# araffin/robotics-rl-srl

Hardware: NVIDIA B200
Metric: env-steps/sec KukaButtonGymEnv-v0 ground_truth @4096 envs/GPU (higher is better)
Workload: dtype f32

## Files before the change

### include/srl_sim.h

```cpp
#ifndef SRL_SIM_H_
#define SRL_SIM_H_

#include <stddef.h>
#include <stdint.h>

#ifdef __cplusplus
extern "C" {
#endif

#define SRL_SIM_ABI_VERSION 1

typedef struct srl_sim srl_sim;

enum srl_env_kind {
    SRL_ENV_KUKA_BUTTON        = 0,
    SRL_ENV_KUKA_RAND_BUTTON   = 1,
    SRL_ENV_KUKA_2BUTTON       = 2,
    SRL_ENV_KUKA_MOVING_BUTTON = 3,
    SRL_ENV_MOBILE             = 4,
    SRL_ENV_MOBILE_2TARGET     = 5,
    SRL_ENV_MOBILE_1D          = 6,
    SRL_ENV_MOBILE_LINE_TARGET = 7
};

typedef struct srl_cfg {
    uint32_t struct_size;
    int32_t  is_discrete;
    int32_t  random_target;
    int32_t  force_down;
    int32_t  shape_reward;
    int32_t  action_joints;
    int32_t  action_repeat;
    int32_t  max_steps;
    int32_t  solver_iterations;
    int32_t  envs_per_warp;
    int32_t  no_auto_reset;
    float    max_distance;
    float    timestep;
    uint32_t prefetch_resets;
    uint64_t global_env_offset;
} srl_cfg;

enum srl_state_field {
    SRL_F_ROBOT_POS     = 0,
    SRL_F_TARGET_POS    = 1,
    SRL_F_STEP_COUNTER  = 2,
    SRL_F_JOINT_POS     = 3,
    SRL_F_JOINT_VEL     = 4,
    SRL_F_EE_CMD        = 5,
    SRL_F_EE_POS        = 6,
    SRL_F_BUTTON_GLIDER = 7,
    SRL_F_COUNTERS      = 8,
    SRL_F_EPISODE_STATS = 9,
    SRL_F_BUTTON_BASE   = 10,
    SRL_F_TWO_BUTTON    = 11,
    SRL_F_NEXT_RECORD   = 12
};

int srl_sim_abi_version(void);

int srl_sim_create(srl_sim** out, int env_kind, int num_envs, int device, const srl_cfg* cfg,
                   const void* model_blob, size_t model_bytes, uint64_t seed);

int srl_sim_reset(srl_sim* sim, const uint8_t* mask, const double* reset_draws, float* obs_out,
                  void* stream);

int srl_sim_step(srl_sim* sim, const void* actions, const float* noise, float* obs_out,
                 float* rew_out, uint8_t* done_out, float* ep_ret_out, int32_t* ep_len_out,
                 void* stream);

int srl_sim_rollout(srl_sim* sim, int T, const void* actions, const float* noise, float* obs_out,
                    float* rew_out, uint8_t* done_out, float* ep_ret_out, int32_t* ep_len_out,
                    void* stream);

int srl_sim_rollout_host(srl_sim* sim, int T, const void* actions, const float* noise,
                         float* obs_out, float* rew_out, uint8_t* done_out);

int srl_sim_prefetch_resets(srl_sim* sim, void* stream);

typedef struct srl_camera {
    float target[3];
    float distance, yaw, pitch, roll;
    float fov;
} srl_camera;
int srl_sim_render(srl_sim* sim, const srl_camera* camera, int width, int height, uint8_t* rgb_out, void* stream);

int srl_sim_get_state(srl_sim* sim, int field, void* dst, size_t bytes);
int srl_sim_set_state(srl_sim* sim, int field, const void* src, size_t bytes);

// ... 16 lines not shown
```

### robotics-rl-srl_b200/csrc/kuka_kernels.cu

```cuda
#include <stdio.h>
#include <stdlib.h>
#include <string.h>
#include <vector>
#include "common.cuh"
#include "kuka_device.cuh"
#include "render_core.h"

struct KukaDev {
    float4* q[3];
    float4* qd[3];
    float4* misc0;
    float4* misc1;
    float4* tgt;
    float4* grip;
    float4* eepos;
    int4*   cnt;
    int4*   cnt2;
    float4* btn2;
    KukaParams P;
    int epw;
    int coop;
};

struct KukaNext {
    float4* q[3]; float4* qd[3];
    float4 *misc0, *misc1, *tgt, *grip, *eepos;
    int4 *cnt, *cnt2;
    float4* btn2;
    uint8_t* valid;
    int32_t* episode;
    uint8_t* progress;
    int helper;
};

namespace {

constexpr float DELTA_V = 0.03f, DELTA_V_CONTINUOUS = 0.0035f, DELTA_THETA = 0.1f;
constexpr double NOISE_STD = 0.01, NOISE_STD_CONTINUOUS = 0.0001, NOISE_STD_JOINTS = 0.002;
constexpr int N_CONTACTS_BEFORE_TERMINATION = 5, N_STEPS_OUTSIDE_SAFETY_SPHERE = 5000, N_RANDOM_ACTIONS_AT_INIT = 5;

template <bool CG, class T>
KK_DEV T ld_state(const T* p) { return CG ? __ldcg(p) : *p; }

template <bool TWOB, bool CG = false, class Arr = KukaDev>
KK_DEV void env_load(const Arr& d, int i, KukaEnv& e) {
#pragma unroll
    for (int k = 0; k < 3; ++k) {
        const float4 a = ld_state<CG>(d.q[k] + i), b = ld_state<CG>(d.qd[k] + i);
        e.q[4 * k] = a.x; e.q[4 * k + 1] = a.y; e.q[4 * k + 2] = a.z; e.q[4 * k + 3] = a.w;
        e.qd[4 * k] = b.x; e.qd[4 * k + 1] = b.y; e.qd[4 * k + 2] = b.z; e.qd[4 * k + 3] = b.w;
    }
    const float4 m0 = ld_state<CG>(d.misc0 + i), m1 = ld_state<CG>(d.misc1 + i), tg = ld_state<CG>(d.tgt + i), gr = ld_state<CG>(d.grip + i),
                 ep = ld_state<CG>(d.eepos + i);
    const int4 c = ld_state<CG>(d.cnt + i), c2 = ld_state<CG>(d.cnt2 + i);
    e.ee[0] = m0.x; e.ee[1] = m0.y; e.ee[2] = m0.z; e.qb = m0.w;
    e.qdb = m1.x; e.bbx = m1.y; e.bby = m1.z; e.ep_ret = m1.w;
    e.tgt[0] = tg.x; e.tgt[1] = tg.y; e.tgt[2] = tg.z; e.bbz = tg.w;
    e.grip[0] = gr.x; e.grip[1] = gr.y; e.grip[2] = gr.z; e.bspeed = gr.w;
    e.eepos[0] = ep.x; e.eepos[1] = ep.y; e.eepos[2] = ep.z;
    e.counter = c.x; e.n_contacts = c.y; e.n_outside = c.z;
    e.terminated = c.w & 1; e.cbutton = (c.w >> 1) & 1; e.ctable = (c.w >> 2) & 1;
    e.episode = (uint32_t)c2.x; e.total_steps = (uint32_t)c2.y; e.ep_len = c2.z;
    e.by64 = __hiloint2double(c2.w, __float_as_int(ep.w));
    e.qb2 = 0.f; e.qdb2 = 0.f; e.bb2x = 0.f; e.bb2y = 0.f; e.n_contacts2 = 0; e.goal_id = 0; e.cany0 = 0; e.cany1 = 0;
// ... 69 lines not shown
        if (P.random_target) {
            if (d17) { e.bb2x = (float)d17[0]; e.bb2y = (float)d17[1]; }
            else {
                const uint4 r = philox4x32_10(P.seed, genv, e.episode, PHILOX_PURPOSE_RESET0);
                e.bb2x = (float)((double)P.btn_base[0] + (double)P.rand_x * (-1.0 + 2.0 * philox_u01(r.x, r.y)));
                e.bb2y = (float)(-(double)P.btn_base[1] + 0.175 * (-1.0 + philox_u01(r.z, r.w)));
            }
        }
        return;
    }
    if (P.random_target) {
        if (d17) { e.bbx = (float)d17[0]; e.bby = (float)d17[1]; e.by64 = d17[1]; }
        else {
            const uint4 r = philox4x32_10(P.seed, genv, e.episode, PHILOX_PURPOSE_RESET0);
            e.bbx = (float)((double)P.btn_base[0] + (double)P.rand_x * (-1.0 + 2.0 * philox_u01(r.x, r.y)));
            e.by64 = (double)P.btn_base[1] + (double)P.rand_y * (-1.0 + 2.0 * philox_u01(r.z, r.w));
            e.bby = (float)e.by64;
        }
    }
}

template <bool TWOB>
KK_DEV void reset_end(const KukaParams& P, KukaEnv& e) {
    e.tgt[0] = e.bbx; e.tgt[1] = e.bby;
    e.tgt[2] = e.bbz + P.glider_z + e.qb + P.target_h;
    if (TWOB) e.tgt[2] = P.two_tgt_z;
    if (TWOB) { e.n_contacts2 = 0; e.goal_id = 0; }
    e.counter = 0; e.n_contacts = 0; e.n_outside = 0; e.terminated = 0;
    e.ep_ret = 0.f; e.ep_len = 0;
    e.episode += 1;
}

enum { KUKA_OP_ROLLOUT = 0, KUKA_OP_RESET = 1, KUKA_OP_SETTLE = 2, KUKA_OP_PREFETCH = 3 };

#ifdef KK_TIMING
__device__ unsigned long long kk_timing[1 << 16];
#define KK_TIMING_RECORD() do { if (lead) kk_timing[(warp * (COOP ? 8 : 32) + slot) & 0xFFFF] = ((unsigned long long)(clock64() - kk_t0) << 32) | dbgf | (helper ? 1u << 18 : 0u); } while (0)
#else
#define KK_TIMING_RECORD() do { } while (0)
#endif
template <bool JOINTS, bool TWOB, bool PREFETCH = false, bool COOP = false>
__global__ void __launch_bounds__(128, 1) kuka_kernel(const __grid_constant__ KukaDev d, int n, int op, int T,
                                                       const void* __restrict__ actions, const float* __restrict__ noise,
                                                       const uint8_t* __restrict__ mask, const double* __restrict__ draws,
                                                       float* __restrict__ obs, float* __restrict__ rew,
                                                       uint8_t* __restrict__ done, float* __restrict__ ep_ret,
                                                       int32_t* __restrict__ ep_len, float* __restrict__ snap, const KukaNext nx) {
    const int lane = threadIdx.x & 31, warp = (blockIdx.x * blockDim.x + threadIdx.x) >> 5;
#ifdef KK_TIMING
    const long long kk_t0 = clock64(); unsigned dbgf = 0u;
#endif
    const int slot = COOP ? lane >> 2 : lane;
    const int u = COOP ? lane & 3 : 0;
    const bool lead = !COOP || u == 0;
    const unsigned gmask = COOP ? 0xFu << (lane & ~3) : 0u;
    extern __shared__ float4 kc_smem[];
    float* const kc_tab = reinterpret_cast<float*>(kc_smem);
    KcScratch sc;
    sc.b = reinterpret_cast<float*>(kc_smem) + ((KC_CONST_WORDS + 31) / 32) * 32 + (8 * (threadIdx.x >> 5) + (lane >> 2)) * KC_ES;
    if constexpr (COOP) {
        kc_fill_const(d.P, kc_tab, threadIdx.x, blockDim.x);
        __syncthreads();
    }
    int i = -1;
    if (slot < d.epw) { i = warp * d.epw + slot; if (i >= n) i = -1; }
    bool helper = false;
    if constexpr (PREFETCH) {
        if (nx.helper && op == KUKA_OP_ROLLOUT && slot == d.epw && slot < (COOP ? 8 : 32)) {
            int pick = -1;
            if (lead) {
                int best = -1;
                for (int k2 = 0; k2 < d.epw; ++k2) {
                    const int j = warp * d.epw + k2;
                    if (j < n && !reinterpret_cast<volatile const uint8_t*>(nx.valid)[j]) {
                        const int pr = nx.progress[j];
                        if (pr > best) { best = pr; pick = j; }
                    }
                }
            }
            if (COOP) pick = __shfl_sync(gmask, pick, lane & ~3);
            if (pick >= 0) { i = pick; helper = true; op = KUKA_OP_PREFETCH; }
        }
    }
    if (i < 0) return;
    if (op == KUKA_OP_RESET && mask && !mask[i]) return;
    if constexpr (PREFETCH) { if (op == KUKA_OP_PREFETCH && !helper && nx.valid[i]) return; }
    const KukaParams& P = d.P;
    const uint64_t genv = P.env_offset + (uint64_t)i;
    const size_t N = (size_t)n;
    KukaEnv e; KukaKin k; KukaContacts ct;
    env_load<TWOB>(d, i, e);
    int nc_reg = 0;
    if constexpr (PREFETCH) {
        __syncwarp();
    }

    int reset_left = 0;
    bool in_reset = false;
    bool pending = false;
    int rep = 0, t = 0;
    int saved_cb = 0, saved_ct = 0, saved_a0 = 0, saved_a1 = 0;
    float dx = 0.f, dy = 0.f, dz = 0.f;
    float qj[JOINTS ? 7 : 1];
#pragma unroll
    for (int j = 0; j < (JOINTS ? 7 : 1); ++j) qj[j] = 0.f;
    const double* d17 = nullptr;
    if (op == KUKA_OP_RESET) {
        d17 = draws ? draws + (size_t)i * 18 : nullptr;
        reset_begin<TWOB>(P, e, d17, genv);
        in_reset = true; reset_left = N_RANDOM_ACTIONS_AT_INIT;
    } else if (op == KUKA_OP_SETTLE) {
#pragma unroll
        for (int j = 0; j < KK_NB; ++j) { e.q[j] = P.snap_q[j]; e.qd[j] = 0.f; }
        e.ee[0] = P.ee_init[0]; e.ee[1] = P.ee_init[1]; e.ee[2] = P.ee_init[2];
        e.qb = 0.f; e.qdb = 0.f; e.bbx = P.btn_base[0]; e.bby = P.btn_base[1]; e.bbz = P.btn_base[2]; e.bspeed = 0.f; e.by64 = 0.0;
        if (TWOB) { e.qb2 = 0.f; e.qdb2 = 0.f; e.bb2x = P.btn_base[0]; e.bb2y = -P.btn_base[1]; }
        in_reset = true; reset_left = 500;
    }
    bool consumed = false;
    bool partial = false;
    int budget = T;
    if constexpr (PREFETCH) {
        if (op == KUKA_OP_PREFETCH) {
            const int prog = helper ? (int)nx.progress[i] : 0;
            if (prog > 0 && nx.episode[i] == (int)e.episode) {
                env_load<TWOB, true>(nx, i, e);
                in_reset = true; reset_left = N_RANDOM_ACTIONS_AT_INIT - prog;
            } else {
                if (helper && lead) nx.episode[i] = (int)e.episode;
                reset_begin<TWOB>(P, e, nullptr, genv);
                in_reset = true; reset_left = N_RANDOM_ACTIONS_AT_INIT;
            }
        }
    }
    for (;;) {
        if constexpr (COOP) {
            KcKinIn kin;
#pragma unroll
            for (int j = 0; j < KK_NB; ++j) kin.q[j] = e.q[j];
            kin.qb = e.qb; kin.qb2 = e.qb2; kin.bbx = e.bbx; kin.bby = e.bby; kin.bbz = e.bbz; kin.bb2x = e.bb2x; kin.bb2y = e.bb2y;
            __syncwarp(gmask);
            const bool near = kc_kinematics<TWOB>(sc, kc_tab, P, kin, u, gmask);
            e.grip[0] = sc[8 * KC_BS + KB_C]; e.grip[1] = sc[8 * KC_BS + KB_C + 1]; e.grip[2] = sc[8 * KC_BS + KB_C + 2];
            e.eepos[0] = sc[6 * KC_BS + KB_P]; e.eepos[1] = sc[6 * KC_BS + KB_P + 1]; e.eepos[2] = sc[6 * KC_BS + KB_P + 2];
            const int fl = near ? (int)sc[KC_OFF_LINK + 6] : 0;
            e.cbutton = fl & 1; e.ctable = (fl >> 1) & 1;
            if (TWOB) { e.cany0 = (fl >> 2) & 1; e.cany1 = (fl >> 3) & 1; }
            nc_reg = near ? (int)sc[KC_OFF_LINK + 7] : 0;
        } else kuka_fk<true, TWOB>(P, e, k, ct);
        const int new_cb = e.cbutton, new_ct = e.ctable, new_a0 = TWOB ? e.cany0 : 0, new_a1 = TWOB ? e.cany1 : 0;
        if (pending) {
            pending = false;
            const size_t off = (size_t)t * N + (size_t)i;
            const float ddx = e.tgt[0] - e.grip[0], ddy = e.tgt[1] - e.grip[1], ddz = e.tgt[2] - e.grip[2];
            const float distance = sqrtf(ddx * ddx + ddy * ddy + ddz * ddz);
            float reward;
            if (TWOB) {
                const int contact = e.goal_id ? saved_a1 : saved_a0;
                reward = 0.f;
                if (e.goal_id) { e.n_contacts2 += contact; reward = contact ? 1.f : 0.f; }
                else {
                    e.n_contacts += contact;
                    if (e.n_contacts >= N_CONTACTS_BEFORE_TERMINATION) { e.goal_id = 1; e.tgt[0] = e.bb2x; e.tgt[1] = e.bb2y; }
                }
                if (distance > P.max_distance || saved_ct) { reward = -1.f; e.n_outside += 1; } else e.n_outside = 0;
                if (saved_ct || e.n_contacts2 >= N_CONTACTS_BEFORE_TERMINATION || e.n_outside >= N_STEPS_OUTSIDE_SAFETY_SPHERE - 1) e.terminated = 1;
                if (P.shape_reward) {
// ... 13 lines not shown
                if (P.is_discrete) reward = -distance;
                else if (e.terminated && reward > 0.f) reward = 50.f;
                else if (e.terminated && reward < 0.f) reward = -250.f;
                else reward = -distance;
            }
            }
            const bool is_done = e.terminated || e.counter > P.max_steps;
#ifdef KK_TIMING
            if (is_done) dbgf |= 1u << 16;
#endif
            e.ep_ret += reward; e.ep_len += 1;
            if (rew && lead) rew[off] = reward;
            if (done && lead) done[off] = is_done ? 1 : 0;
            if (is_done && lead) {
                if (ep_ret) ep_ret[off] = e.ep_ret;
                if (ep_len) ep_len[off] = e.ep_len;
            }
            if (is_done && P.auto_reset) {
                if constexpr (PREFETCH) {
                    if (op == KUKA_OP_ROLLOUT) {
                        int rec = 0;
                        if (lead && reinterpret_cast<volatile const uint8_t*>(nx.valid)[i]) {
                            __threadfence();
                            rec = reinterpret_cast<volatile const int32_t*>(nx.episode)[i] == (int)e.episode ? 2 : 1;
                        }
                        if (COOP) rec = __shfl_sync(gmask, rec, lane & ~3);
#ifdef KK_TIMING
                        if (rec == 2) dbgf |= 1u << 17;
#endif
                        if (rec == 2) {
                            const uint32_t total_steps = e.total_steps;
                            env_load<TWOB, true>(nx, i, e);
                            e.total_steps = total_steps;
                            __threadfence();
                            if (COOP) __syncwarp(gmask);
                        }
                        if (rec && lead) reinterpret_cast<volatile uint8_t*>(nx.valid)[i] = 0;
                        if (rec == 2) {
                            saved_cb = e.cbutton; saved_ct = e.ctable;
                            if (TWOB) { saved_a0 = e.cany0; saved_a1 = e.cany1; }
                            consumed = true; in_reset = true; reset_left = 0;
                            continue;
                        }
                    }
                }
                d17 = nullptr;
                reset_begin<TWOB>(P, e, nullptr, genv);
                in_reset = true; reset_left = N_RANDOM_ACTIONS_AT_INIT;
                continue;
            }
            if (obs && lead) { float* o = obs + 3 * off; o[0] = e.grip[0] - e.tgt[0]; o[1] = e.grip[1] - e.tgt[1]; o[2] = e.grip[2] - e.tgt[2]; }
            ++t;
        }
        if (in_reset && reset_left == 0) {
            in_reset = false;
            if (op == KUKA_OP_SETTLE) {
                if (lead) {
                    for (int j = 0; j < KK_NB; ++j) { snap[j] = e.q[j]; snap[KK_NB + j] = e.qd[j]; }
                    snap[24] = e.ee[0]; snap[25] = e.ee[1]; snap[26] = e.ee[2]; snap[27] = e.qb; snap[28] = e.qdb;
                }
                return;
            }
            if (!(PREFETCH && consumed)) reset_end<TWOB>(P, e);
            consumed = false;
            if (obs && lead && op != KUKA_OP_PREFETCH) {
                float* o = obs + 3 * (op == KUKA_OP_RESET ? (size_t)i : (size_t)t * N + (size_t)i);
                o[0] = e.grip[0] - e.tgt[0]; o[1] = e.grip[1] - e.tgt[1]; o[2] = e.grip[2] - e.tgt[2];
            }
            if (op == KUKA_OP_ROLLOUT) ++t;
        }
        if (!in_reset && (op != KUKA_OP_ROLLOUT || t >= T)) break;
        bool armed;
        if (in_reset) {
            if (op == KUKA_OP_SETTLE) { dx = dy = dz = 0.f; }
            else reset_action(P, d17, genv, e.episode, N_RANDOM_ACTIONS_AT_INIT - reset_left, dx, dy, dz);
            if (JOINTS) {
#pragma unroll
                for (int j = 0; j < 7; ++j) qj[JOINTS ? j : 0] = P.qinit[j] + dx;
            }
            --reset_left;
            armed = false;
        } else {
            if (rep == 0) {
                const size_t off = (size_t)t * N + (size_t)i;
                float nz;
                if (noise) nz = __ldg(noise + off);
                else {
                    const uint4 r = philox4x32_10(P.seed, genv, e.total_steps, PHILOX_PURPOSE_NOISE);
                    const double u1 = philox_u01(r.x, r.y), u2 = philox_u01(r.z, r.w);
                    nz = (float)((JOINTS ? NOISE_STD_JOINTS : P.is_discrete ? NOISE_STD : NOISE_STD_CONTINUOUS) * sqrt(-2.0 * log(1.0 - u1)) * cos(6.283185307179586 * u2));
                }
                dx = dy = dz = 0.f;
                uint4 ra = make_uint4(0, 0, 0, 0);
                if (!actions) ra = philox4x32_10(P.seed, genv, e.total_steps, PHILOX_PURPOSE_ACTION);
                if (JOINTS) {
                    float a7[7];
                    if (actions) {
// ... 23 lines not shown
                    if (actions) {
                        const float* ap = reinterpret_cast<const float*>(actions) + 3 * off;
                        a0 = __ldg(ap); a1 = __ldg(ap + 1); a2 = __ldg(ap + 2);
                    } else {
                        a0 = (float)((double)ra.x * (2.0 / 4294967296.0) - 1.0);
                        a1 = (float)((double)ra.y * (2.0 / 4294967296.0) - 1.0);
                        a2 = (float)((double)ra.z * (2.0 / 4294967296.0) - 1.0);
                    }
                    const float dv = DELTA_V_CONTINUOUS + nz;
                    dx = a0 * dv; dy = a1 * dv;
                    dz = P.force_down ? -fabsf(a2 * dv) : a2 * dv;
                }
                e.total_steps += 1;
                if (P.moving_button) {
                    if (e.by64 > 0.3 || e.by64 < -0.3) e.bspeed = -e.bspeed;
                    e.by64 = __dadd_rn(e.by64, e.bspeed > 0.f ? 0.001 : -0.001);
                    e.tgt[1] = (float)e.by64;
                    e.bbx = e.tgt[0]; e.bby = e.tgt[1]; e.bbz = e.tgt[2] - P.target_h;
                }
            }
            armed = true;
        }
        if (!JOINTS) apply_ee_delta(P, e, dx, dy, dz);
        saved_cb = new_cb; saved_ct = new_ct; saved_a0 = new_a0; saved_a1 = new_a1;
#ifdef KK_TIMING
        kuka_physics_step<JOINTS, TWOB, COOP>(P, e, k, ct, armed, qj, sc, u, gmask, nc_reg, &dbgf);
#else
        kuka_physics_step<JOINTS, TWOB, COOP>(P, e, k, ct, armed, qj, sc, u, gmask, nc_reg);
#endif
        if constexpr (PREFETCH) { if (helper && --budget <= 0 && reset_left > 0) { partial = true; break; } }
        if (!in_reset) {
            if (e.terminated || e.counter > P.max_steps) { pending = true; rep = 0; }
            else { e.counter += 1; if (++rep == P.action_repeat) { pending = true; rep = 0; } }
        }
    }
    e.cbutton = saved_cb; e.ctable = saved_ct;
    if (TWOB) { e.cany0 = saved_a0; e.cany1 = saved_a1; }
    KK_TIMING_RECORD();
    if constexpr (PREFETCH) {
        if (op == KUKA_OP_PREFETCH) {
            if (!lead) return;
            env_store<TWOB>(nx, i, e);
            if (partial) { nx.progress[i] = (uint8_t)(N_RANDOM_ACTIONS_AT_INIT - reset_left); return; }
            nx.episode[i] = (int)e.episode - 1;
            nx.progress[i] = 0;
            __threadfence();
            reinterpret_cast<volatile uint8_t*>(nx.valid)[i] = 1;
            return;
        }
    }
    if (lead) env_store<TWOB>(d, i, e);
}

template <bool TWOB>
__global__ void kuka_prims_kernel(const __grid_constant__ KukaDev d, int n, float* __restrict__ prims, int* __restrict__ counts) {
    const int i = blockIdx.x * blockDim.x + threadIdx.x;
    if (i >= n) return;
    const KukaParams& P = d.P;
    KukaEnv e; KukaKin k; KukaContacts ct;
    env_load<TWOB>(d, i, e);
    float Rb[KK_NB][9]; f3 pb[KK_NB];
    {
        float R[9] = {1.f, 0.f, 0.f, 0.f, 1.f, 0.f, 0.f, 0.f, 1.f}, R7[9]; f3 p = mk3(P.base[0], P.base[1], P.base[2]), p7 = p;
        for (int t = 0; t < 9; ++t) R7[t] = R[t];
        for (int b = 0; b < KK_NB; ++b) {
            if (b == 10) { for (int t = 0; t < 9; ++t) R[t] = R7[t]; p = p7; }
            const float ox = P.org[b][0], oy = P.org[b][1], oz = P.org[b][2];
            p = mk3(p.x + R[0] * ox + R[1] * oy + R[2] * oz, p.y + R[3] * ox + R[4] * oy + R[5] * oz, p.z + R[6] * ox + R[7] * oy + R[8] * oz);
            float sn, cs; sincosf(e.q[b], &sn, &cs);
            const float t = 1.f - cs, ax = P.axis[b][0], ay = P.axis[b][1], az = P.axis[b][2];
            const float Q[9] = {cs + t * ax * ax, t * ax * ay - sn * az, t * ax * az + sn * ay, t * ax * ay + sn * az, cs + t * ay * ay, t * ay * az - sn * ax,
                                t * ax * az - sn * ay, t * ay * az + sn * ax, cs + t * az * az};
            float B[9], Rn[9];
            for (int r = 0; r < 3; ++r) for (int c = 0; c < 3; ++c) B[3 * r + c] = P.rot[b][3 * r] * Q[c] + P.rot[b][3 * r + 1] * Q[3 + c] + P.rot[b][3 * r + 2] * Q[6 + c];
            for (int r = 0; r < 3; ++r) for (int c = 0; c < 3; ++c) Rn[3 * r + c] = R[3 * r] * B[c] + R[3 * r + 1] * B[3 + c] + R[3 * r + 2] * B[6 + c];
            for (int t2 = 0; t2 < 9; ++t2) { R[t2] = Rn[t2]; Rb[b][t2] = Rn[t2]; }
            pb[b] = p;
            if (b == 7) { for (int t2 = 0; t2 < 9; ++t2) R7[t2] = R[t2]; p7 = p; }
        }
    }
// ... 155 lines not shown

int kuka_alloc(srl_sim* s, const void* blob, size_t bytes) {
    KukaDev* d = new KukaDev();
    memset(d, 0, sizeof(*d));
    s->kuka = d;
    if (!fill_params(blob, bytes, s, d->P)) return 1;
    const size_t N = (size_t)s->n;
    float4** f4[] = {&d->q[0], &d->q[1], &d->q[2], &d->qd[0], &d->qd[1], &d->qd[2], &d->misc0, &d->misc1, &d->tgt, &d->grip, &d->eepos};
    for (float4** p : f4) { SRL_CUDA_OK(cudaMalloc(p, N * sizeof(float4))); SRL_CUDA_OK(cudaMemset(*p, 0, N * sizeof(float4))); }
    SRL_CUDA_OK(cudaMalloc(&d->cnt, N * sizeof(int4))); SRL_CUDA_OK(cudaMemset(d->cnt, 0, N * sizeof(int4)));
    SRL_CUDA_OK(cudaMalloc(&d->cnt2, N * sizeof(int4))); SRL_CUDA_OK(cudaMemset(d->cnt2, 0, N * sizeof(int4)));
    SRL_CUDA_OK(cudaMalloc(&d->btn2, N * sizeof(float4))); SRL_CUDA_OK(cudaMemset(d->btn2, 0, N * sizeof(float4)));
    int sms = 148;
    cudaDeviceGetAttribute(&sms, cudaDevAttrMultiProcessorCount, s->device);
    int epw = s->cfg.envs_per_warp;
    if (epw <= 0) { epw = (int)((N + (size_t)sms * 4 - 1) / ((size_t)sms * 4)); }
    if (epw < 1) epw = 1;
    if (epw > 32) epw = 32;
    d->epw = epw;
    d->coop = epw <= 8 ? 1 : 0;
    if (const char* co = getenv("SRL_KUKA_COOP")) d->coop = (atoi(co) != 0 && epw <= 8) ? 1 : 0;
    float* snap = nullptr;
    SRL_CUDA_OK(cudaMalloc(&snap, 32 * sizeof(float)));
    { const int save_epw = d->epw; d->epw = 1;
      KUKA_LAUNCH(d, 1, 32, 0, 1, KUKA_OP_SETTLE, 0, nullptr, nullptr, nullptr, nullptr, nullptr, nullptr, nullptr, nullptr, nullptr, snap);
      d->epw = save_epw; }
    SRL_CUDA_OK(cudaGetLastError());
    float h[32];
    SRL_CUDA_OK(cudaMemcpy(h, snap, sizeof(h), cudaMemcpyDeviceToHost));
    cudaFree(snap);
    for (int i = 0; i < KK_NB; ++i) { d->P.snap_q[i] = h[i]; d->P.snap_qd[i] = h[KK_NB + i]; }
    d->P.snap_ee[0] = h[24]; d->P.snap_ee[1] = h[25]; d->P.snap_ee[2] = h[26]; d->P.snap_qb = h[27]; d->P.snap_qdb = h[28];
    s->launches += 1;
    if (s->cfg.prefetch_resets && s->auto_reset && !d->P.two_buttons && !d->P.action_joints) {
        KukaNextHost* nh = new KukaNextHost();
        memset(nh, 0, sizeof(*nh));
        s->kuka_next = nh;
        KukaNext& nx = nh->nx;
        float4** g4[] = {&nx.q[0], &nx.q[1], &nx.q[2], &nx.qd[0], &nx.qd[1], &nx.qd[2], &nx.misc0, &nx.misc1, &nx.tgt, &nx.grip, &nx.eepos, &nx.btn2};
        for (float4** p : g4) { SRL_CUDA_OK(cudaMalloc(p, N * sizeof(float4))); SRL_CUDA_OK(cudaMemset(*p, 0, N * sizeof(float4))); }
        SRL_CUDA_OK(cudaMalloc(&nx.cnt, N * sizeof(int4))); SRL_CUDA_OK(cudaMemset(nx.cnt, 0, N * sizeof(int4)));
        SRL_CUDA_OK(cudaMalloc(&nx.cnt2, N * sizeof(int4))); SRL_CUDA_OK(cudaMemset(nx.cnt2, 0, N * sizeof(int4)));
        SRL_CUDA_OK(cudaMalloc(&nx.valid, N)); SRL_CUDA_OK(cudaMemset(nx.valid, 0, N));
        SRL_CUDA_OK(cudaMalloc(&nx.episode, N * sizeof(int32_t))); SRL_CUDA_OK(cudaMemset(nx.episode, 0xff, N * sizeof(int32_t)));
        SRL_CUDA_OK(cudaMalloc(&nx.progress, N)); SRL_CUDA_OK(cudaMemset(nx.progress, 0, N));
        SRL_CUDA_OK(cudaEventCreateWithFlags(&s->pf_ev, cudaEventDisableTiming));
        SRL_CUDA_OK(cudaEventCreateWithFlags(&s->roll_ev, cudaEventDisableTiming));
        nh->enabled = true;
    }
    return 0;
}

void kuka_free(srl_sim* s) {
    KukaDev* d = s->kuka;
    if (!d) return;
    for (int k = 0; k < 3; ++k) { cudaFree(d->q[k]); cudaFree(d->qd[k]); }
    cudaFree(d->misc0); cudaFree(d->misc1); cudaFree(d->tgt); cudaFree(d->grip); cudaFree(d->eepos); cudaFree(d->cnt); cudaFree(d->cnt2); cudaFree(d->btn2);
    delete d;
    s->kuka = nullptr;
    if (KukaNextHost* nh = static_cast<KukaNextHost*>(s->kuka_next)) {
        KukaNext& nx = nh->nx;
        for (int k = 0; k < 3; ++k) { cudaFree(nx.q[k]); cudaFree(nx.qd[k]); }
        cudaFree(nx.misc0); cudaFree(nx.misc1); cudaFree(nx.tgt); cudaFree(nx.grip); cudaFree(nx.eepos); cudaFree(nx.cnt); cudaFree(nx.cnt2);
        cudaFree(nx.btn2); cudaFree(nx.valid); cudaFree(nx.episode); cudaFree(nx.progress);
        delete nh;
        s->kuka_next = nullptr;
        if (s->pf_ev) cudaEventDestroy(s->pf_ev);
        if (s->roll_ev) cudaEventDestroy(s->roll_ev);
    }
}

int kuka_launch_reset(srl_sim* s, const uint8_t* mask, const double* draws, float* obs, cudaStream_t st) {
    KukaDev* d = s->kuka;
    int grid, block; grid_for(s, d, grid, block);
    KUKA_LAUNCH(d, grid, block, st, s->n, KUKA_OP_RESET, 0, nullptr, nullptr, mask, draws, obs, nullptr, nullptr, nullptr, nullptr, nullptr);
    SRL_CUDA_OK(cudaGetLastError());
    return 0;
}

int kuka_launch_rollout(srl_sim* s, int T, const void* actions, const float* noise, float* obs, float* rew, uint8_t* done,
                        float* ep_ret, int32_t* ep_len, cudaStream_t st) {
    KukaDev* d = s->kuka;
    int grid, block; grid_for(s, d, grid, block);
    const KukaNextHost* nh = static_cast<const KukaNextHost*>(s->kuka_next);
    if (nh && nh->enabled) {
        cudaStreamCaptureStatus cap = cudaStreamCaptureStatusNone;
        cudaStreamIsCapturing(st, &cap);
        const bool capturing = cap != cudaStreamCaptureStatusNone;
        if (s->pf_pending && !capturing) { SRL_CUDA_OK(cudaStreamWaitEvent(st, s->pf_ev, 0)); s->pf_pending = false; }
        KukaNext nx = nh->nx;
        nx.helper = 1;
        if (d->coop) SRL_CUDA_OK((kuka_launch_inst<false, false, true, true>(d, grid, block, st, s->n, KUKA_OP_ROLLOUT, T, actions, noise, nullptr, nullptr, obs, rew, done, ep_ret, ep_len, nullptr, nx)));
        else SRL_CUDA_OK((kuka_launch_inst<false, false, true, false>(d, grid, block, st, s->n, KUKA_OP_ROLLOUT, T, actions, noise, nullptr, nullptr, obs, rew, done, ep_ret, ep_len, nullptr, nx)));
        if (!capturing) { SRL_CUDA_OK(cudaEventRecord(s->roll_ev, st)); s->roll_ev_valid = true; }
    }
    else
        KUKA_LAUNCH(d, grid, block, st, s->n, KUKA_OP_ROLLOUT, T, actions, noise, nullptr, nullptr, obs, rew, done, ep_ret, ep_len, nullptr);
// ... 85 lines not shown
        SRL_CUDA_OK(pull(a, d->btn2));
        SRL_CUDA_OK(cudaMemcpy(ia.data(), d->cnt, N * sizeof(int4), cudaMemcpyDeviceToHost));
        SRL_CUDA_OK(cudaMemcpy(ib.data(), d->cnt2, N * sizeof(int4), cudaMemcpyDeviceToHost));
        for (size_t i = 0; i < N; ++i) {
            D[8 * i] = d->P.two_buttons ? ia[i].y : 0; D[8 * i + 1] = d->P.two_buttons ? ib[i].w : 0; D[8 * i + 2] = (ia[i].w >> 5) & 1;
            D[8 * i + 3] = a[i].z; D[8 * i + 4] = a[i].w; D[8 * i + 5] = d->P.btn_base[2]; D[8 * i + 6] = a[i].x; D[8 * i + 7] = a[i].y;
        }
        return 0;
    }
    case SRL_F_EPISODE_STATS: {
        if (!need(2, 8)) return 1;
        SRL_CUDA_OK(pull(b, d->misc1));
        SRL_CUDA_OK(cudaMemcpy(ia.data(), d->cnt2, N * sizeof(int4), cudaMemcpyDeviceToHost));
        for (size_t i = 0; i < N; ++i) { D[2 * i] = b[i].w; D[2 * i + 1] = (double)ia[i].z; }
        return 0;
    }
#ifdef KK_TIMING
    case 99: {
        if (cudaMemcpyFromSymbol(dst, kk_timing, bytes < sizeof(kk_timing) ? bytes : sizeof(kk_timing)) != cudaSuccess) return 1;
        return 0;
    }
#endif
    case SRL_F_NEXT_RECORD: {
        if (!need(3, 4)) return 1;
        const KukaNextHost* nh = static_cast<const KukaNextHost*>(s->kuka_next);
        for (size_t i = 0; i < N; ++i) { I[3 * i] = 0; I[3 * i + 1] = 0; I[3 * i + 2] = -1; }
        if (nh && nh->enabled) {
            std::vector<uint8_t> va(N), pr(N); std::vector<int32_t> ep(N);
            SRL_CUDA_OK(cudaMemcpy(va.data(), nh->nx.valid, N, cudaMemcpyDeviceToHost));
            SRL_CUDA_OK(cudaMemcpy(pr.data(), nh->nx.progress, N, cudaMemcpyDeviceToHost));
            SRL_CUDA_OK(cudaMemcpy(ep.data(), nh->nx.episode, N * sizeof(int32_t), cudaMemcpyDeviceToHost));
            for (size_t i = 0; i < N; ++i) { I[3 * i] = va[i]; I[3 * i + 1] = pr[i]; I[3 * i + 2] = ep[i]; }
        }
        return 0;
    }
    default:
        srl_set_error("get_state: unknown field %d", field);
        return 1;
    }
}

int kuka_set_state(srl_sim* s, int field, const void* src, size_t bytes) {
    KukaDev* d = s->kuka;
    const size_t N = (size_t)s->n;
    SRL_CUDA_OK(cudaDeviceSynchronize());
    auto need = [&](size_t width, size_t elem) { if (bytes != N * width * elem) { srl_set_error("set_state: size mismatch"); return false; } return true; };
    const double* D = (const double*)src; const int32_t* I = (const int32_t*)src;
    std::vector<float4> a(N), b(N), c(N);
    auto pull = [&](std::vector<float4>& v, const float4* p) { return cudaMemcpy(v.data(), p, N * sizeof(float4), cudaMemcpyDeviceToHost); };
    auto push = [&](const std::vector<float4>& v, float4* p) { return cudaMemcpy(p, v.data(), N * sizeof(float4), cudaMemcpyHostToDevice); };
    switch (field) {
    case SRL_F_JOINT_POS: case SRL_F_JOINT_VEL: {
        if (!need(KK_NB, 8)) return 1;
        float4* const* dst = field == SRL_F_JOINT_POS ? d->q : d->qd;
        for (size_t i = 0; i < N; ++i) {
            a[i] = make_float4((float)D[12 * i], (float)D[12 * i + 1], (float)D[12 * i + 2], (float)D[12 * i + 3]);
            b[i] = make_float4((float)D[12 * i + 4], (float)D[12 * i + 5], (float)D[12 * i + 6], (float)D[12 * i + 7]);
            c[i] = make_float4((float)D[12 * i + 8], (float)D[12 * i + 9], (float)D[12 * i + 10], (float)D[12 * i + 11]);
        }
        SRL_CUDA_OK(push(a, dst[0])); SRL_CUDA_OK(push(b, dst[1])); SRL_CUDA_OK(push(c, dst[2]));
        return 0;
    }
    case SRL_F_EE_CMD:
        if (!need(3, 8)) return 1;
        SRL_CUDA_OK(pull(a, d->misc0));
        for (size_t i = 0; i < N; ++i) { a[i].x = (float)D[3 * i]; a[i].y = (float)D[3 * i + 1]; a[i].z = (float)D[3 * i + 2]; }
// ... 37 lines not shown
```

### robotics-rl-srl_b200/rl_baselines/ppo2.py

```python
import json
import os
import time

import numpy as np
import torch
import torch.nn as nn

from srl_sim.vec_env import BatchedSRLVecEnv

PPO2_DEFAULTS = dict(n_steps=128, ent_coef=0.01, learning_rate=2.5e-4, vf_coef=0.5, max_grad_norm=0.5, gamma=0.99, lam=0.95,
                     nminibatches=4, noptepochs=4, cliprange=0.2)


class MlpPolicy(nn.Module):

    def __init__(self, obs_dim, n_actions=None, action_dim=None):
        super().__init__()
        self.discrete = n_actions is not None
        out = n_actions if self.discrete else action_dim

        def tower(last, gain):
            layers = [nn.Linear(obs_dim, 64), nn.Tanh(), nn.Linear(64, 64), nn.Tanh(), nn.Linear(64, last)]
            for m in layers:
                if isinstance(m, nn.Linear):
# ... 57 lines not shown
    def stats(mean, var, count):
        return torch.cat([count.reshape(1), count * mean, count * (var + mean * mean)])
    d = norm.mean.numel()
    s = stats(norm.mean, norm.var, norm.count)
    all_reduce_sum(s)
    s = s - (world - 1) * stats(*prior)
    count, mean = s[0], s[1:1 + d] / s[0]
    norm.count.copy_(count)
    norm.mean.copy_(mean)
    norm.var.copy_(torch.clamp(s[1 + d:] / count - mean * mean, min=0.0))


def allreduce_mean_gradients(params, dist, world):
    grads = [p.grad for p in params]
    flat = torch.cat([g.reshape(-1) for g in grads])
    dist.all_reduce(flat)
    flat.div_(world)
    off = 0
    for g in grads:
        n = g.numel()
        g.copy_(flat[off:off + n].view_as(g))
        off += n


def train(env_id, num_envs, num_timesteps, seed=0, env_kwargs=None, log_dir=None, device=0, hyperparams=None, verbose=1, cuda_graph=True,
          phase_times=None, fused_act=None, prefetch_resets=None, episode_window=40, fused_update=None):
    hp = dict(PPO2_DEFAULTS); hp.update(hyperparams or {})
    torch.manual_seed(seed)
    env_kwargs = dict(env_kwargs or {})
    dist, rank, world = _dist_world()
    if prefetch_resets is None:
        from srl_sim.backend import default_backend
        prefetch_resets = default_backend(device).on_gpu
    if prefetch_resets:
        env_kwargs["prefetch_resets"] = True
    if env_kwargs.get("srl_model", "ground_truth") != "ground_truth":
        raise ValueError("ppo2.train supports srl_model='ground_truth' only (got %r)" % env_kwargs["srl_model"])
    import types
    from rl_baselines.utils import createTensorEnvs, save_obs_rms
    env = createTensorEnvs(types.SimpleNamespace(env=env_id, num_cpu=num_envs, seed=seed, device=device), env_kwargs=env_kwargs,
                           global_env_offset=rank * num_envs)
    on_gpu = env.backend.on_gpu
    dev = env.backend.torch_device if on_gpu else torch.device("cpu")
    e_obs, e_rew, e_done, e_ep_ret, e_ep_len = [x if on_gpu else torch.from_numpy(x) for x in (env._obs, env._rew, env._done, env._ep_ret, env._ep_len)]
    D = env.observation_space.shape[0]
    if env.is_discrete:
        policy = MlpPolicy(D, n_actions=env.action_space.n).to(dev)
    else:
        policy = MlpPolicy(D, action_dim=env.action_space.shape[0]).to(dev)
    params = list(policy.parameters())
    if dist is not None:
        for p in params:
            dist.broadcast(p.data, 0)
        torch.manual_seed(seed + rank)
    N, T = num_envs, hp["n_steps"]
    graph_update = bool(cuda_graph and on_gpu and dist is None and (T * N) % hp["nminibatches"] == 0)
    if graph_update:
        lr_t = torch.tensor(float(hp["learning_rate"]), device=dev, dtype=torch.float32)
        opt = torch.optim.Adam(params, lr=lr_t, eps=1e-5, capturable=True)
    else:
        opt = torch.optim.Adam(params, lr=hp["learning_rate"], eps=1e-5)
    norm = RunningNorm(D, dev)
    n_updates = max(1, int(num_timesteps) // (N * T * world))
    if log_dir and rank == 0:
        os.makedirs(log_dir, exist_ok=True)
        with open(os.path.join(log_dir, "args.json"), "w") as f:
            json.dump(dict(env=env_id, algo="ppo2", num_cpu=N, num_timesteps=num_timesteps, seed=seed, srl_model="ground_truth", **hp), f)
        with open(os.path.join(log_dir, "env_globals.json"), "w") as f:
# ... 257 lines not shown
```

### robotics-rl-srl_b200/srl_sim/_abi.py

```python
import ctypes
import os
from ctypes import (POINTER, Structure, byref, c_char_p, c_double, c_float, c_int, c_int32,
                    c_size_t, c_uint8, c_uint32, c_uint64, c_void_p)

import numpy as np

ABI_VERSION = 1

ENV_KINDS = {
    "KukaButtonGymEnv-v0": 0,
    "KukaRandButtonGymEnv-v0": 1,
    "Kuka2ButtonGymEnv-v0": 2,
    "KukaMovingButtonGymEnv-v0": 3,
    "MobileRobotGymEnv-v0": 4,
    "MobileRobot2TargetGymEnv-v0": 5,
    "MobileRobot1DGymEnv-v0": 6,
    "MobileRobotLineTargetGymEnv-v0": 7,
}

F_ROBOT_POS, F_TARGET_POS, F_STEP_COUNTER, F_JOINT_POS, F_JOINT_VEL, F_EE_CMD, F_EE_POS, \
    F_BUTTON_GLIDER, F_COUNTERS, F_EPISODE_STATS, F_BUTTON_BASE, F_TWO_BUTTON, F_NEXT_RECORD = range(13)

_FIELD_SPEC = {
    F_ROBOT_POS: (np.float64, 3), F_TARGET_POS: (np.float64, 3), F_STEP_COUNTER: (np.int32, 1),
    F_JOINT_POS: (np.float64, 12), F_JOINT_VEL: (np.float64, 12), F_EE_CMD: (np.float64, 3),
    F_EE_POS: (np.float64, 3), F_BUTTON_GLIDER: (np.float64, 2), F_COUNTERS: (np.int32, 4),
    F_EPISODE_STATS: (np.float64, 2), F_BUTTON_BASE: (np.float64, 3), F_TWO_BUTTON: (np.float64, 8), F_NEXT_RECORD: (np.int32, 3),
}

MOBILE_RESET_DRAWS = 6
KUKA_RESET_DRAWS = 18


class SrlCfg(Structure):
    _fields_ = [
        ("struct_size", c_uint32),
        ("is_discrete", c_int32),
        ("random_target", c_int32),
        ("force_down", c_int32),
        ("shape_reward", c_int32),
        ("action_joints", c_int32),
        ("action_repeat", c_int32),
        ("max_steps", c_int32),
        ("solver_iterations", c_int32),
        ("envs_per_warp", c_int32),
        ("no_auto_reset", c_int32),
        ("max_distance", c_float),
        ("timestep", c_float),
        ("prefetch_resets", c_uint32),
        ("global_env_offset", c_uint64),
    ]


class SimError(RuntimeError):
    pass


_EXPORTS = [
    ("srl_sim_abi_version", c_int, []),
    ("srl_sim_create", c_int, [POINTER(c_void_p), c_int, c_int, c_int, POINTER(SrlCfg), c_void_p, c_size_t, c_uint64]),
    ("srl_sim_reset", c_int, [c_void_p, c_void_p, c_void_p, c_void_p, c_void_p]),
# ... 55 lines not shown
        return msg.decode("utf-8", "replace") if msg else ""

    def check(self, rc, what):
        if rc != 0:
            msg = self.last_error()
            if rc == 2:
                raise ValueError(msg)
            raise SimError("%s failed (rc=%d): %s" % (what, rc, msg))


class Sim(object):

    def __init__(self, library, env_kind, num_envs, device, seed=0, model_blob=None, **cfg):
        self.library = library
        self._lib = library.lib
        self.handle = c_void_p()
        if isinstance(env_kind, str):
            env_kind = ENV_KINDS[env_kind]
        self.env_kind = env_kind
        c = SrlCfg()
        c.struct_size = ctypes.sizeof(SrlCfg)
        c.is_discrete = int(cfg.pop("is_discrete", True))
        c.random_target = int(cfg.pop("random_target", False))
        c.force_down = int(cfg.pop("force_down", True))
        c.shape_reward = int(cfg.pop("shape_reward", False))
        c.action_joints = int(cfg.pop("action_joints", False))
        c.action_repeat = int(cfg.pop("action_repeat", 1))
        c.max_steps = int(cfg.pop("max_steps", 0))
        c.solver_iterations = int(cfg.pop("solver_iterations", 0))
        c.envs_per_warp = int(cfg.pop("envs_per_warp", 0))
        c.no_auto_reset = int(cfg.pop("no_auto_reset", False))
        c.max_distance = float(cfg.pop("max_distance", 0.8))
        c.timestep = float(cfg.pop("timestep", 0.0))
        c.prefetch_resets = int(bool(cfg.pop("prefetch_resets", False)))
        c.global_env_offset = int(cfg.pop("global_env_offset", 0))
        if cfg:
            raise TypeError("unknown cfg keys: %s" % sorted(cfg))
        self.cfg = c
        blob_ptr, blob_len = None, 0
        if model_blob is not None:
            self._blob = np.ascontiguousarray(model_blob)
            blob_ptr, blob_len = self._blob.ctypes.data, self._blob.nbytes
        rc = self._lib.srl_sim_create(byref(self.handle), env_kind, int(num_envs), int(device), byref(c),
                                      blob_ptr, blob_len, int(seed) & 0xFFFFFFFFFFFFFFFF)
        library.check(rc, "srl_sim_create")
        self.num_envs = self._lib.srl_sim_num_envs(self.handle)
        self.obs_dim = self._lib.srl_sim_obs_dim(self.handle)
        self.action_dim = self._lib.srl_sim_action_dim(self.handle)
        self.is_discrete = bool(c.is_discrete)
        self.device = device

    def close(self):
        if self.handle:
            self._lib.srl_sim_destroy(self.handle)
            self.handle = c_void_p()

    def __del__(self):
        try:
            self.close()
        except Exception:
            pass

    def reset(self, mask=None, reset_draws=None, obs_out=None, stream=None):
        rc = self._lib.srl_sim_reset(self.handle, _ptr(mask), _ptr(reset_draws), _ptr(obs_out), stream)
        self.library.check(rc, "srl_sim_reset")

    def step(self, actions, noise=None, obs_out=None, rew_out=None, done_out=None, ep_ret_out=None,
# ... 59 lines not shown
```

Before: 98.93 million.

## Enable reset prefetch by default, chain helper records, prefetch step inputs to L1

```diff
diff --git a/include/srl_sim.h b/include/srl_sim.h
--- a/include/srl_sim.h
+++ b/include/srl_sim.h
@@ -41,6 +41,8 @@
     uint64_t global_env_offset;
 } srl_cfg;
 
+enum srl_prefetch_mode { SRL_PREFETCH_DEFAULT = 0, SRL_PREFETCH_ON = 1, SRL_PREFETCH_OFF = 2 };
+
 enum srl_state_field {
     SRL_F_ROBOT_POS     = 0,
     SRL_F_TARGET_POS    = 1,
@@ -54,7 +56,8 @@
     SRL_F_EPISODE_STATS = 9,
     SRL_F_BUTTON_BASE   = 10,
     SRL_F_TWO_BUTTON    = 11,
-    SRL_F_NEXT_RECORD   = 12
+    SRL_F_NEXT_RECORD   = 12,
+    SRL_F_RECORD_HITS   = 13
 };
 
 int srl_sim_abi_version(void);
diff --git a/robotics-rl-srl_b200/csrc/kuka_kernels.cu b/robotics-rl-srl_b200/csrc/kuka_kernels.cu
--- a/robotics-rl-srl_b200/csrc/kuka_kernels.cu
+++ b/robotics-rl-srl_b200/csrc/kuka_kernels.cu
@@ -30,6 +30,7 @@
     uint8_t* valid;
     int32_t* episode;
     uint8_t* progress;
+    int32_t* hits;
     int helper;
 };
 
@@ -165,6 +166,30 @@
 }
 
 enum { KUKA_OP_ROLLOUT = 0, KUKA_OP_RESET = 1, KUKA_OP_SETTLE = 2, KUKA_OP_PREFETCH = 3 };
+
+KK_DEV int record_pick(const KukaNext& nx, int warp, int epw, int n) {
+    int pick = -1, best = -1;
+    for (int k2 = 0; k2 < epw; ++k2) {
+        const int j = warp * epw + k2;
+        if (j < n && !reinterpret_cast<volatile const uint8_t*>(nx.valid)[j]) {
+            const int pr = nx.progress[j];
+            if (pr > best) { best = pr; pick = j; }
+        }
+    }
+    if (pick >= 0) __threadfence();
+    return pick;
+}
+
+template <bool TWOB>
+KK_DEV void record_publish(const KukaNext& nx, int i, const KukaEnv& e) {
+    env_store<TWOB>(nx, i, e);
+    nx.episode[i] = (int)e.episode - 1;
+    nx.progress[i] = 0;
+    __threadfence();
+    reinterpret_cast<volatile uint8_t*>(nx.valid)[i] = 1;
+}
+
+KK_DEV void prefetch_l1(const void* p) { asm volatile("prefetch.global.L1 [%0];" ::"l"(p)); }
 
 #ifdef KK_TIMING
 __device__ unsigned long long kk_timing[1 << 16];
@@ -200,17 +225,7 @@
     bool helper = false;
     if constexpr (PREFETCH) {
         if (nx.helper && op == KUKA_OP_ROLLOUT && slot == d.epw && slot < (COOP ? 8 : 32)) {
-            int pick = -1;
-            if (lead) {
-                int best = -1;
-                for (int k2 = 0; k2 < d.epw; ++k2) {
-                    const int j = warp * d.epw + k2;
-                    if (j < n && !reinterpret_cast<volatile const uint8_t*>(nx.valid)[j]) {
-                        const int pr = nx.progress[j];
-                        if (pr > best) { best = pr; pick = j; }
-                    }
-                }
-            }
+            int pick = lead ? record_pick(nx, warp, d.epw, n) : -1;
             if (COOP) pick = __shfl_sync(gmask, pick, lane & ~3);
             if (pick >= 0) { i = pick; helper = true; op = KUKA_OP_PREFETCH; }
         }
@@ -219,7 +234,7 @@
     if (op == KUKA_OP_RESET && mask && !mask[i]) return;
     if constexpr (PREFETCH) { if (op == KUKA_OP_PREFETCH && !helper && nx.valid[i]) return; }
     const KukaParams& P = d.P;
-    const uint64_t genv = P.env_offset + (uint64_t)i;
+    uint64_t genv = P.env_offset + (uint64_t)i;
     const size_t N = (size_t)n;
     KukaEnv e; KukaKin k; KukaContacts ct;
     env_load<TWOB>(d, i, e);
@@ -250,22 +265,37 @@
         if (TWOB) { e.qb2 = 0.f; e.qdb2 = 0.f; e.bb2x = P.btn_base[0]; e.bb2y = -P.btn_base[1]; }
         in_reset = true; reset_left = 500;
     }
+    auto record_begin = [&]() {
+        const int prog = helper ? (int)nx.progress[i] : 0;
+        const int ep = reinterpret_cast<volatile const int32_t*>(nx.episode)[i];
+        if (prog > 0 && ep == (int)e.episode) {
+            env_load<TWOB, true>(nx, i, e);
+            in_reset = true; reset_left = N_RANDOM_ACTIONS_AT_INIT - prog;
+        } else {
+            if (ep > (int)e.episode) e.episode = (uint32_t)ep;
+            if (helper && lead) nx.episode[i] = (int)e.episode;
+            reset_begin<TWOB>(P, e, nullptr, genv);
+            in_reset = true; reset_left = N_RANDOM_ACTIONS_AT_INIT;
+        }
+    };
     bool consumed = false;
     bool partial = false;
     int budget = T;
     if constexpr (PREFETCH) {
         if (op == KUKA_OP_PREFETCH) {
-            const int prog = helper ? (int)nx.progress[i] : 0;
-            if (prog > 0 && nx.episode[i] == (int)e.episode) {
-                env_load<TWOB, true>(nx, i, e);
-                in_reset = true; reset_left = N_RANDOM_ACTIONS_AT_INIT - prog;
-            } else {
-                if (helper && lead) nx.episode[i] = (int)e.episode;
-                reset_begin<TWOB>(P, e, nullptr, genv);
-                in_reset = true; reset_left = N_RANDOM_ACTIONS_AT_INIT;
-            }
-        }
-    }
+            record_begin();
+        }
+    }
+    auto prefetch_step_inputs = [&](int ts) {
+        const size_t o = (size_t)ts * N + (size_t)i;
+        if (noise) prefetch_l1(noise + o);
+        if (actions) {
+            if (JOINTS) { prefetch_l1(reinterpret_cast<const float*>(actions) + 7 * o); prefetch_l1(reinterpret_cast<const float*>(actions) + 7 * o + 6); }
+            else if (P.is_discrete) prefetch_l1(reinterpret_cast<const int32_t*>(actions) + o);
+            else { prefetch_l1(reinterpret_cast<const float*>(actions) + 3 * o); prefetch_l1(reinterpret_cast<const float*>(actions) + 3 * o + 2); }
+        }
+    };
+    if (op == KUKA_OP_ROLLOUT && T > 0) prefetch_step_inputs(0);
     for (;;) {
         if constexpr (COOP) {
             KcKinIn kin;
@@ -345,6 +375,12 @@
                             const uint32_t total_steps = e.total_steps;
                             env_load<TWOB, true>(nx, i, e);
                             e.total_steps = total_steps;
+                        }
+                        if (rec) {
+                            if (lead) {
+                                reinterpret_cast<volatile int32_t*>(nx.episode)[i] = (int)e.episode + (rec == 2 ? 0 : 1);
+                                if (rec == 2) nx.hits[i] += 1;
+                            }
                             __threadfence();
                             if (COOP) __syncwarp(gmask);
                         }
@@ -376,6 +412,19 @@
             }
             if (!(PREFETCH && consumed)) reset_end<TWOB>(P, e);
             consumed = false;
+            if constexpr (PREFETCH) {
+                if (helper) {
+                    e.cbutton = saved_cb; e.ctable = saved_ct;
+                    if (lead) record_publish<TWOB>(nx, i, e);
+                    int pick = (lead && budget > 0) ? record_pick(nx, warp, d.epw, n) : -1;
+                    if (COOP) pick = __shfl_sync(gmask, pick, lane & ~3);
+                    if (pick < 0) { KK_TIMING_RECORD(); return; }
+                    i = pick; genv = P.env_offset + (uint64_t)i;
+                    env_load<TWOB>(d, i, e);
+                    record_begin();
+                    continue;
+                }
+            }
             if (obs && lead && op != KUKA_OP_PREFETCH) {
                 float* o = obs + 3 * (op == KUKA_OP_RESET ? (size_t)i : (size_t)t * N + (size_t)i);
                 o[0] = e.grip[0] - e.tgt[0]; o[1] = e.grip[1] - e.tgt[1]; o[2] = e.grip[2] - e.tgt[2];
@@ -465,6 +514,7 @@
         if (!in_reset) {
             if (e.terminated || e.counter > P.max_steps) { pending = true; rep = 0; }
             else { e.counter += 1; if (++rep == P.action_repeat) { pending = true; rep = 0; } }
+            if (pending && op == KUKA_OP_ROLLOUT && t + 1 < T) prefetch_step_inputs(t + 1);
         }
     }
     e.cbutton = saved_cb; e.ctable = saved_ct;
@@ -473,12 +523,8 @@
     if constexpr (PREFETCH) {
         if (op == KUKA_OP_PREFETCH) {
             if (!lead) return;
-            env_store<TWOB>(nx, i, e);
-            if (partial) { nx.progress[i] = (uint8_t)(N_RANDOM_ACTIONS_AT_INIT - reset_left); return; }
-            nx.episode[i] = (int)e.episode - 1;
-            nx.progress[i] = 0;
-            __threadfence();
-            reinterpret_cast<volatile uint8_t*>(nx.valid)[i] = 1;
+            if (partial) { env_store<TWOB>(nx, i, e); nx.progress[i] = (uint8_t)(N_RANDOM_ACTIONS_AT_INIT - reset_left); return; }
+            record_publish<TWOB>(nx, i, e);
             return;
         }
     }
@@ -700,7 +746,7 @@
     for (int i = 0; i < KK_NB; ++i) { d->P.snap_q[i] = h[i]; d->P.snap_qd[i] = h[KK_NB + i]; }
     d->P.snap_ee[0] = h[24]; d->P.snap_ee[1] = h[25]; d->P.snap_ee[2] = h[26]; d->P.snap_qb = h[27]; d->P.snap_qdb = h[28];
     s->launches += 1;
-    if (s->cfg.prefetch_resets && s->auto_reset && !d->P.two_buttons && !d->P.action_joints) {
+    if (s->cfg.prefetch_resets != SRL_PREFETCH_OFF && s->auto_reset && !d->P.two_buttons && !d->P.action_joints) {
         KukaNextHost* nh = new KukaNextHost();
         memset(nh, 0, sizeof(*nh));
         s->kuka_next = nh;
@@ -712,6 +758,7 @@
         SRL_CUDA_OK(cudaMalloc(&nx.valid, N)); SRL_CUDA_OK(cudaMemset(nx.valid, 0, N));
         SRL_CUDA_OK(cudaMalloc(&nx.episode, N * sizeof(int32_t))); SRL_CUDA_OK(cudaMemset(nx.episode, 0xff, N * sizeof(int32_t)));
         SRL_CUDA_OK(cudaMalloc(&nx.progress, N)); SRL_CUDA_OK(cudaMemset(nx.progress, 0, N));
+        SRL_CUDA_OK(cudaMalloc(&nx.hits, N * sizeof(int32_t))); SRL_CUDA_OK(cudaMemset(nx.hits, 0, N * sizeof(int32_t)));
         SRL_CUDA_OK(cudaEventCreateWithFlags(&s->pf_ev, cudaEventDisableTiming));
         SRL_CUDA_OK(cudaEventCreateWithFlags(&s->roll_ev, cudaEventDisableTiming));
         nh->enabled = true;
@@ -730,7 +777,7 @@
         KukaNext& nx = nh->nx;
         for (int k = 0; k < 3; ++k) { cudaFree(nx.q[k]); cudaFree(nx.qd[k]); }
         cudaFree(nx.misc0); cudaFree(nx.misc1); cudaFree(nx.tgt); cudaFree(nx.grip); cudaFree(nx.eepos); cudaFree(nx.cnt); cudaFree(nx.cnt2);
-        cudaFree(nx.btn2); cudaFree(nx.valid); cudaFree(nx.episode); cudaFree(nx.progress);
+        cudaFree(nx.btn2); cudaFree(nx.valid); cudaFree(nx.episode); cudaFree(nx.progress); cudaFree(nx.hits);
         delete nh;
         s->kuka_next = nullptr;
         if (s->pf_ev) cudaEventDestroy(s->pf_ev);
@@ -882,6 +929,13 @@
             SRL_CUDA_OK(cudaMemcpy(ep.data(), nh->nx.episode, N * sizeof(int32_t), cudaMemcpyDeviceToHost));
             for (size_t i = 0; i < N; ++i) { I[3 * i] = va[i]; I[3 * i + 1] = pr[i]; I[3 * i + 2] = ep[i]; }
         }
+        return 0;
+    }
+    case SRL_F_RECORD_HITS: {
+        if (!need(1, 4)) return 1;
+        const KukaNextHost* nh = static_cast<const KukaNextHost*>(s->kuka_next);
+        if (nh && nh->enabled) SRL_CUDA_OK(cudaMemcpy(I, nh->nx.hits, N * sizeof(int32_t), cudaMemcpyDeviceToHost));
+        else memset(I, 0, N * sizeof(int32_t));
         return 0;
     }
     default:
diff --git a/robotics-rl-srl_b200/rl_baselines/ppo2.py b/robotics-rl-srl_b200/rl_baselines/ppo2.py
--- a/robotics-rl-srl_b200/rl_baselines/ppo2.py
+++ b/robotics-rl-srl_b200/rl_baselines/ppo2.py
@@ -113,8 +113,7 @@
     if prefetch_resets is None:
         from srl_sim.backend import default_backend
         prefetch_resets = default_backend(device).on_gpu
-    if prefetch_resets:
-        env_kwargs["prefetch_resets"] = True
+    env_kwargs["prefetch_resets"] = bool(prefetch_resets)
     if env_kwargs.get("srl_model", "ground_truth") != "ground_truth":
         raise ValueError("ppo2.train supports srl_model='ground_truth' only (got %r)" % env_kwargs["srl_model"])
     import types
diff --git a/robotics-rl-srl_b200/srl_sim/_abi.py b/robotics-rl-srl_b200/srl_sim/_abi.py
--- a/robotics-rl-srl_b200/srl_sim/_abi.py
+++ b/robotics-rl-srl_b200/srl_sim/_abi.py
@@ -19,14 +19,17 @@
 }
 
 F_ROBOT_POS, F_TARGET_POS, F_STEP_COUNTER, F_JOINT_POS, F_JOINT_VEL, F_EE_CMD, F_EE_POS, \
-    F_BUTTON_GLIDER, F_COUNTERS, F_EPISODE_STATS, F_BUTTON_BASE, F_TWO_BUTTON, F_NEXT_RECORD = range(13)
+    F_BUTTON_GLIDER, F_COUNTERS, F_EPISODE_STATS, F_BUTTON_BASE, F_TWO_BUTTON, F_NEXT_RECORD, F_RECORD_HITS = range(14)
 
 _FIELD_SPEC = {
     F_ROBOT_POS: (np.float64, 3), F_TARGET_POS: (np.float64, 3), F_STEP_COUNTER: (np.int32, 1),
     F_JOINT_POS: (np.float64, 12), F_JOINT_VEL: (np.float64, 12), F_EE_CMD: (np.float64, 3),
     F_EE_POS: (np.float64, 3), F_BUTTON_GLIDER: (np.float64, 2), F_COUNTERS: (np.int32, 4),
     F_EPISODE_STATS: (np.float64, 2), F_BUTTON_BASE: (np.float64, 3), F_TWO_BUTTON: (np.float64, 8), F_NEXT_RECORD: (np.int32, 3),
+    F_RECORD_HITS: (np.int32, 1),
 }
+
+PREFETCH_DEFAULT, PREFETCH_ON, PREFETCH_OFF = range(3)
 
 MOBILE_RESET_DRAWS = 6
 KUKA_RESET_DRAWS = 18
@@ -148,7 +151,8 @@
         c.no_auto_reset = int(cfg.pop("no_auto_reset", False))
         c.max_distance = float(cfg.pop("max_distance", 0.8))
         c.timestep = float(cfg.pop("timestep", 0.0))
-        c.prefetch_resets = int(bool(cfg.pop("prefetch_resets", False)))
+        pf = cfg.pop("prefetch_resets", None)
+        c.prefetch_resets = PREFETCH_DEFAULT if pf is None else PREFETCH_ON if pf else PREFETCH_OFF
         c.global_env_offset = int(cfg.pop("global_env_offset", 0))
         if cfg:
             raise TypeError("unknown cfg keys: %s" % sorted(cfg))
```

New measurement: 87.74 million (median of 6 runs). 0.887x the previous value.
